# rafaelcgon/2D-GP

Hardware: AMD Instinct MI355X
Metric: posterior grid points/sec (fit+predict), N_train=4096, div-free 2D kernel (higher is better)
Workload: dtype f64 (variance GEMM as exact int8 Ozaki-II); 1 GPU; df kernel, N_train=4096, 256x256 grid per GPU, fit+predict (mean+variance); n_train=4096, grid_per_gpu=256x256, points_total=65536, parallelism=grid-sharded x1, factor local, kstar_ahead=False

## Files before the change

### 2d-gp_amd/csrc/gp2d.hip

```cpp
#include "common.hpp"
#ifndef GP2D_RELEASE
#error "libgp2d.so is built with -DGP2D_RELEASE=1 (python __graft_entry__.py build)"
#endif
#include "assemble.hpp"
#include "gemm_f64.hpp"
#include "factor.hpp"
#include "predict.hpp"
#include "fields.hpp"
#include "grad.hpp"
#include "postcov.hpp"
#include "predict_host.hpp"
#include "ozaki.hpp"
#include "ozaki_host.hpp"
#include "factor_host.hpp"
#include "lml.hpp"
#include "lml_host.hpp"
#include "dfact.hpp"
#include "order.hpp"
#include "../../include/gp2d.h"

#include <dlfcn.h>

#include <algorithm>
#include <cstdlib>
// ... 1067 lines not shown
  GP2D_REQUIRE(bufs_ok, "ozaki: NULL buffer");
  GP2D_REQUIRE(nmod_out != nullptr, "ozaki: nmod_out is NULL");
  return 0;
}

static int prepare_finish(int nmod, const gp2d_kernel_t* k, int pw, int pb, const double* W, int64_t n, WRows wr,
                          int8_t* wres, double* rowscale, bool fused, int* nmod_out, hipStream_t s) {
  OzakiConsts oc;
  GP2D_CHECK(make_ozaki_consts(nmod, k, oc, pw, pb));
  if (fused) {
    ozaki_w_scale_kernel<<<(unsigned)n, 256, 0, s>>>(W, n, wr, pw, rowscale, nullptr, oc.M, oc.sB, 1);
    GP2D_CHECK(check_launch("ozaki_w_scale_kernel"));
  } else {
    ozaki_rowscale_final_kernel<<<(unsigned)((n + 255) / 256), 256, 0, s>>>(rowscale, n, oc.M, oc.sB);
    GP2D_CHECK(check_launch("ozaki_rowscale_final_kernel"));
  }
  GP2D_CHECK(launch_w_res(W, n, wr, oc, wres, rowscale, s));
  *nmod_out = nmod;
  return 0;
}

int gp2d_ozaki_prepare(const double* W, int64_t n, int64_t ldw, const gp2d_kernel_t* k, int wbits, int kbits,
                       int8_t* wres, double* rowscale, int* nmod_out, void* stream) {
  GP2D_CHECK(prepare_args(k, wbits, kbits, n, true, nmod_out));
  const int pw = ozaki_wbits(wbits), pb = ozaki_kbits(kbits);
  hipStream_t s = S(stream);
  double* l1 = reinterpret_cast<double*>(wres);
  ozaki_w_scale_kernel<<<(unsigned)n, 256, 0, s>>>(W, n, WRows{ldw}, pw, rowscale, l1, 0.0, 0, 0);
  GP2D_CHECK(check_launch("ozaki_w_scale_kernel"));
  std::vector<double> hl1((size_t)n), hs((size_t)n);
  if (hipMemcpyAsync(hl1.data(), l1, sizeof(double) * n, hipMemcpyDeviceToHost, s) != hipSuccess ||
      hipMemcpyAsync(hs.data(), rowscale, sizeof(double) * n, hipMemcpyDeviceToHost, s) != hipSuccess ||
      hipStreamSynchronize(s) != hipSuccess) {
    set_error("ozaki: reading the row bounds failed");
    return -1;
  }
  int sB = 0;
  {
    OzakiConsts probe;
    GP2D_CHECK(make_ozaki_consts(1, k, probe, pw, pb));
    sB = probe.sB;
  }
  const double sq = 2.0 * std::sqrt(gp2d_kernel_diag(k));
  double bmax = 1.0;
  for (int64_t i = 0; i < n; ++i) {
    const double a = std::ldexp(hl1[i] * 1.01, pb - 1);
    const double b = std::ldexp(sq, (int)hs[i] + sB) + std::ldexp((double)n, pb - 2) + hl1[i] + (double)n;
    bmax = std::max(bmax, std::min(a, b));
  }
  const int nmod = ozaki_nmod_bits(std::log2(bmax));
  GP2D_REQUIRE(nmod > 0, "ozaki: row bound exceeds the modulus table");
  return prepare_finish(nmod, k, pw, pb, W, n, WRows{ldw}, wres, rowscale, false, nmod_out, s);
}

static int prepare_apriori(const double* W, int64_t n, WRows wr, const gp2d_kernel_t* k, double diag_add,
                           int wbits, int kbits, int8_t* wres, double* rowscale, int* nmod_out, hipStream_t s) {
  GP2D_CHECK(prepare_args(k, wbits, kbits, n, W != nullptr && wres != nullptr && rowscale != nullptr, nmod_out));
  const int pw = ozaki_wbits(wbits), pb = ozaki_kbits(kbits);
  const int nmod = gp2d_ozaki_nmod_apriori(n, k, diag_add, pw, pb);
  GP2D_REQUIRE(nmod > 0, "ozaki: a-priori bound exceeds the modulus table");
  return prepare_finish(nmod, k, pw, pb, W, n, wr, wres, rowscale, true, nmod_out, s);
}

int gp2d_ozaki_prepare_async(const double* W, int64_t n, int64_t ldw, const gp2d_kernel_t* k, double diag_add,
                             int wbits, int kbits, int8_t* wres, double* rowscale, int* nmod_out, void* stream) {
  GP2D_REQUIRE(ldw >= n, "ozaki: ldw must be >= n");
  return prepare_apriori(W, n, WRows{ldw}, k, diag_add, wbits, kbits, wres, rowscale, nmod_out, S(stream));
}

int gp2d_ozaki_prepare_packed(const double* packed, int64_t n, const gp2d_kernel_t* k, double diag_add, int wbits,
                              int kbits, int8_t* wres, double* rowscale, int* nmod_out, void* stream) {
  GP2D_REQUIRE(n % NB == 0, "ozaki: n must be a multiple of 128 (the packing's row blocks)");
  return prepare_apriori(packed, n, WRows{0}, k, diag_add, wbits, kbits, wres, rowscale, nmod_out, S(stream));
}

size_t gp2d_ozaki_guard_workspace(int64_t n) {
  if (n <= 0) return 0;
  return 2 * sizeof(double) * (size_t)((n + OZ_GUARD_RSEG - 1) / OZ_GUARD_RSEG) * (size_t)n;
}

int gp2d_ozaki_guard(const double* W, int64_t n, int64_t ldw, int64_t ntr, int64_t npad, double diag_add,
                     double* stats, void* work, size_t work_bytes, void* stream) {
  GP2D_REQUIRE(W && stats && n > 0 && ldw >= n && ntr >= 1 && npad >= ntr && (n == npad || n == 2 * npad),
               "ozaki_guard: bad arguments");
  GP2D_REQUIRE(std::isfinite(diag_add), "ozaki_guard: the diagonal addition (noise + jitter) must be finite");
  GP2D_REQUIRE(work != nullptr && work_bytes >= gp2d_ozaki_guard_workspace(n), "ozaki_guard: workspace too small");
  hipStream_t s = S(stream);
  const int64_t nseg = (n + OZ_GUARD_RSEG - 1) / OZ_GUARD_RSEG;
  double* psum = static_cast<double*>(work);
  double* pmax = psum + nseg * n;
  ozaki_guard_colsq_kernel<<<dim3((unsigned)((n + 255) / 256), (unsigned)nseg), 256, 0, s>>>(W, n, ldw, psum, pmax);
  GP2D_CHECK(check_launch("ozaki_guard_colsq_kernel"));
  ozaki_guard_finish_kernel<<<1, 1024, 0, s>>>(psum, pmax, n, nseg, ntr, npad, diag_add, stats);
  return check_launch("ozaki_guard_finish_kernel");
}

static constexpr double OZ_GUARD_A = 2.87e-15, OZ_GUARD_B = 3.58e-14;
double gp2d_ozaki_error_model(double kss, double vmin, int wbits, int kbits) {
  if (!(kss > 0.0)) return INFINITY;
  if (!(vmin > 0.0)) return INFINITY;
  const double X = kss / vmin;
  return OZ_GUARD_A * std::ldexp(1.0, OZ_PW - ozaki_wbits(wbits)) * X * std::sqrt(X) +
         OZ_GUARD_B * std::ldexp(1.0, OZ_PB - ozaki_kbits(kbits)) * X;
}

int gp2d_ozaki_guard_bits(double kss, double vmin, double target, int* wbits, int* kbits) {
  if (!(target > 0.0) || wbits == nullptr || kbits == nullptr) return -1;
  for (int tot = OZ_PW + OZ_PB; tot <= OZ_PW_MAX + OZ_PB_MAX; ++tot) {
    int bw = 0, bk = 0;
    double best = INFINITY;
    for (int pb = OZ_PB; pb <= OZ_PB_MAX; ++pb) {
      const int pw = tot - pb;
      if (pw < OZ_PW || pw > OZ_PW_MAX) continue;
      const double e = gp2d_ozaki_error_model(kss, vmin, pw, pb);
      if (e <= target && e < best) { best = e; bw = pw; bk = pb; }
    }
    if (bw) {
      *wbits = bw;
      *kbits = bk;
      return 1;
    }
  }
  return 0;
}

static int g_oz_skip = 1;
void gp2d_ozaki_set_skip(int on) { g_oz_skip = on ? 1 : 0; }

size_t gp2d_predict_ozaki_workspace(int64_t n, int64_t chunk) {
  return OzakiWork(n, chunk, ozaki_nmod_for(n), true).total;
}

size_t gp2d_predict_ozaki_workspace_nmod(int64_t n, int64_t chunk, int nmod) {
  if (nmod <= 0 || nmod > ozaki_nmod_for(n)) return 0;
  return std::max(OzakiWork(n, chunk, nmod, true).total, OzakiWork(n, chunk, nmod, false).total);
}

size_t gp2d_predict_ozaki_planes_workspace(int64_t n, int64_t chunk) {
  return OzakiWork(n, chunk, ozaki_nmod_for(n), false).total;
}

struct OzakiChunk {
  int64_t cv, cp, ncols;
  const double* xg;
  dim3 kgrid;
  OzakiChunk(const double* xg0, int64_t m, int64_t c0, int64_t chunk, int64_t ntr_pad, const gp2d_kernel_t* k)
      : cv(std::min<int64_t>(chunk, m - c0)), cp(round_up(cv, IBN)), ncols(2 * cp), xg(xg0 + point_dim(k) * c0),
        kgrid((unsigned)((ntr_pad + OZ_KS_T - 1) / OZ_KS_T), (unsigned)(cp / OZ_KS_P)) {}
};

static int launch_kstar(const OzakiChunk& c, hipStream_t s, const double* xtr, int64_t ntr, int64_t npad,
                        const VecParams& vp, const double* alpha, const OzakiConsts& oc, int8_t* bres, double* pm,
                        uint8_t* flags) {
  if ((uint64_t)(2 * npad) * (uint64_t)c.ncols < (1ull << 31))
    ozaki_kstar_kernel<true><<<c.kgrid, 256, 0, s>>>(xtr, ntr, npad, c.xg, c.cv, c.cp, vp, alpha, oc, bres, pm, flags);
  else
    ozaki_kstar_kernel<false><<<c.kgrid, 256, 0, s>>>(xtr, ntr, npad, c.xg, c.cv, c.cp, vp, alpha, oc, bres, pm, flags);
  return check_launch("ozaki_kstar_kernel");
}

static int predict_ozaki_impl(const int8_t* wres, const double* rowscale, int nmod, int kbits, int64_t n,
                              const double* alpha, const double* xtr, int64_t ntr,
                              int64_t ntr_pad, const double* xg, int64_t m, const gp2d_kernel_t* k, int var_mode,
                              double noise, int compute_var, double* mean, double* var,
                              const int64_t* out_order, int64_t chunk, const OzakiWork& lay, void* work,
                              const KstarBuf* pre, const int8_t* pre_base, hipStream_t s) {
  const auto [bres, cres, pm, P, flags, skip] = lay.at(work);
  OzakiConsts oc;
  GP2D_CHECK(make_ozaki_consts(nmod, k, oc, OZ_PW, ozaki_kbits(kbits)));
  const int nm = oc.nmod;
  GP2D_REQUIRE(n < 131072, "ozaki: the int8 GEMM epilogue needs n < 131072 (N_train < 65536)");
  const int64_t nmseg = (ntr_pad + OZ_KS_T - 1) / OZ_KS_T;
  const int64_t npseg = (n + OZ_CRT_ROWS - 1) / OZ_CRT_ROWS;
  const double kss = gp2d_kernel_diag(k);
  const double add = (var_mode == GP2D_VAR_LATENT) ? 0.0 : noise;
  const int clip = (var_mode == GP2D_VAR_CLIPPED);
  const VecParams vp = make_vec_params(k);
  OzakiConsts oc_mean_only = oc;
  oc_mean_only.nmod = 0;
  int64_t ci = 0;
  for (int64_t c0 = 0; c0 < m; c0 += chunk, ++ci) {
    const OzakiChunk c(xg, m, c0, chunk, ntr_pad, k);
    const int64_t cv = c.cv, cp = c.cp, ncols = c.ncols;
    const int8_t* B = pre ? pre_base + pre->planes_at(ci) : bres;
    const uint8_t* F = pre ? reinterpret_cast<const uint8_t*>(pre_base + pre->flags_at(ci)) : flags;
    const size_t bplane = (size_t)ncols * n;
    const bool inline_planes = compute_var && !pre;
    GP2D_CHECK(launch_kstar(c, s, xtr, ntr, ntr_pad, vp, alpha, inline_planes ? oc : oc_mean_only,
                            pre ? nullptr : bres, pm, inline_planes ? flags : nullptr));
    const int nbj = (int)(ncols / IBN), kslabs = (int)(n / IBK);
    const bool use_skip = compute_var && g_oz_skip && kslabs <= (1 << 20);
    int* slist = skip;
    int* scnt = skip + (int64_t)nbj * kslabs;
    if (use_skip) {
      ozaki_slab_list_kernel<<<(unsigned)nbj, 64, 0, s>>>(F, (int)(ntr_pad / OZ_KS_T), nbj, kslabs, slist, scnt);
      GP2D_CHECK(check_launch("ozaki_slab_list_kernel"));
    }
    if (compute_var) {
      const double nv = 2.0 * (double)ntr;
      TimedLaunch timed(s, 2.0 * (double)cv * nv * nv);
      const int zper = (n <= kIgemmZBatchMaxN) ? nm : 1;
      for (int l0 = 0; l0 < nm; l0 += zper) {
        const int nz = std::min(zper, nm - l0);
        IgemmZ zb{(int64_t)n * n, (int64_t)bplane, (int64_t)n * ncols, {}};
        for (int u = 0; u < nz; ++u) zb.m[u] = oc.m[l0 + u];
        constexpr int tbn = 256, nst = I_NSTAGE;
        const dim3 ggrid((unsigned)(ncols / tbn), (unsigned)(n / IBM), (unsigned)nz);
        const int8_t* Al = wres + (size_t)l0 * n * n;
        const int8_t* Bl = B + (size_t)l0 * bplane;
        uint8_t* Cl = cres + (size_t)l0 * n * ncols;
        igemm_nt_mod_kernel<tbn, nst><<<ggrid, 2 * tbn, 0, s>>>(Al, Bl, Cl, n, (int)n, (int)ncols, (int)n, 1, oc.m[l0],
                                                                (int)(cp / IBN), (int)(ntr_pad / IBK),
                                                                use_skip ? slist : nullptr, use_skip ? scnt : nullptr,
                                                                zb);
        GP2D_CHECK(check_launch("igemm_nt_mod_kernel"));
      }
      timed.stop();
      const dim3 cgrid((unsigned)((ncols + OZ_CRT_BCOLS - 1) / OZ_CRT_BCOLS), (unsigned)npseg);
      ozaki_crt_colsq_kernel<<<cgrid, 256, 0, s>>>(cres, n, ncols, oc, rowscale, P);
      GP2D_CHECK(check_launch("ozaki_crt_colsq_kernel"));
    }
    GP2D_CHECK(launch_finalize({pm, nmseg, P, npseg, ncols, cp, cv, c0, m, kss, add, clip, compute_var, mean, var,
                                out_order}, s));
  }
  return 0;
}

static int predict_ozaki_args(const gp2d_kernel_t* k, int64_t n, int64_t ntr_pad, int64_t chunk, int var_mode,
                              bool ptrs_ok, int64_t m, int nmod, int kbits, const OzakiWork& lay, const void* work,
                              size_t work_bytes) {
  GP2D_CHECK(validate_ozaki_kernel(k));
  GP2D_REQUIRE(n == 2 * ntr_pad && n % IBM == 0, "ozaki: n must equal 2·ntr_pad and be a multiple of 256");
  GP2D_REQUIRE(chunk > 0 && chunk % (IBN / 2) == 0, "ozaki: chunk must be a positive multiple of 128");
  GP2D_REQUIRE(var_mode >= 0 && var_mode <= 2, "predict: bad var_mode");
  GP2D_REQUIRE(ptrs_ok, "ozaki_planes: alpha and the K* planes are required");
  if (m <= 0) return 1;
  GP2D_REQUIRE(nmod > 0 && nmod <= ozaki_nmod_for(n), "ozaki: nmod exceeds the moduli table");
  GP2D_REQUIRE(work != nullptr && work_bytes >= lay.total, "ozaki: workspace too small");
  return valid_bits(0, kbits);
}

int gp2d_predict_ozaki(const int8_t* wres, const double* rowscale, int nmod, int kbits, int64_t n, const double* alpha,
                       const double* xtr,
                       int64_t ntr, int64_t ntr_pad, const double* xg, int64_t m, const gp2d_kernel_t* k,
                       int var_mode, double noise, int compute_var, double* mean, double* var,
                       const int64_t* out_order, int64_t chunk, void* work, size_t work_bytes, void* stream) {
  const OzakiWork lay(n, chunk, nmod, true);
  const int rc = predict_ozaki_args(k, n, ntr_pad, chunk, var_mode, true, m, nmod, kbits, lay, work, work_bytes);
  if (rc != 0) return rc < 0 ? rc : 0;
  return predict_ozaki_impl(wres, rowscale, nmod, kbits, n, alpha, xtr, ntr, ntr_pad, xg, m, k, var_mode, noise,
                            compute_var, mean, var, out_order, chunk, lay, work, nullptr, nullptr, S(stream));
}

int gp2d_ozaki_nmod_apriori(int64_t n, const gp2d_kernel_t* k, double diag_add, int wbits, int kbits) {
  if (validate_ozaki_kernel(k) != 0 || n <= 0 || valid_bits(wbits, kbits) != 0) return -1;
  const int pw = ozaki_wbits(wbits), pb = ozaki_kbits(kbits);
  const double kss = gp2d_kernel_diag(k);
  const double dmin = (1.0 - std::ldexp(1.0, -40)) / std::sqrt(kss + diag_add);
  const int smax = pw - 1 - (int)std::floor(std::log2(dmin));
  OzakiConsts probe;
  if (make_ozaki_consts(1, k, probe, pw, pb) != 0) return -1;
  const double sq = 2.0 * std::sqrt(kss);
  const double b = std::ldexp(sq, smax + probe.sB) + std::ldexp((double)n, pb - 2) + std::ldexp((double)n, pw) +
                   (double)n;
  const double a_id = 1.01 * std::ldexp(1.0, pw + pb - 2);
  return ozaki_nmod_bits(std::log2(std::max(b, a_id)));
}

size_t gp2d_ozaki_kstar_bytes(int64_t n, int64_t m, int64_t chunk, int nmod) {
  if (n <= 0 || m <= 0 || chunk <= 0 || nmod <= 0) return 0;
  return (size_t)((m + chunk - 1) / chunk) * KstarBuf(n, chunk, nmod).stride;
}

int gp2d_ozaki_kstar(const double* xtr, int64_t ntr, int64_t ntr_pad, const double* xg, int64_t m,
                     const gp2d_kernel_t* k, int nmod, int kbits, int64_t chunk, int8_t* bres, size_t bres_bytes,
                     void* stream) {
  GP2D_CHECK(validate_ozaki_kernel(k));
  const int64_t n = 2 * ntr_pad;
  GP2D_REQUIRE(ntr_pad > 0 && n % IBM == 0 && ntr <= ntr_pad, "ozaki_kstar: 2·ntr_pad must be a multiple of 256");
  GP2D_REQUIRE(chunk > 0 && chunk % (IBN / 2) == 0, "ozaki_kstar: chunk must be a positive multiple of 128");
  GP2D_REQUIRE(nmod > 0 && nmod <= OZ_MAXMOD, "ozaki_kstar: bad number of moduli");
  GP2D_CHECK(valid_bits(0, kbits));
  if (m <= 0) return 0;
  GP2D_REQUIRE(bres != nullptr && bres_bytes >= gp2d_ozaki_kstar_bytes(n, m, chunk, nmod),
               "ozaki_kstar: plane buffer too small");
  OzakiConsts oc;
  GP2D_CHECK(make_ozaki_consts(nmod, k, oc, OZ_PW, ozaki_kbits(kbits)));
  const VecParams vp = make_vec_params(k);
  const KstarBuf buf(n, chunk, nmod);
  hipStream_t s = S(stream);
  int64_t ci = 0;
  for (int64_t c0 = 0; c0 < m; c0 += chunk, ++ci) {
    const OzakiChunk c(xg, m, c0, chunk, ntr_pad, k);
    GP2D_CHECK(launch_kstar(c, s, xtr, ntr, ntr_pad, vp, nullptr, oc, bres + buf.planes_at(ci), nullptr,
                            reinterpret_cast<uint8_t*>(bres + buf.flags_at(ci))));
  }
  return 0;
}

int gp2d_predict_ozaki_planes(const int8_t* wres, const double* rowscale, int nmod, int kbits, int64_t n,
                              const double* alpha, const double* xtr, int64_t ntr, int64_t ntr_pad, const double* xg,
                              int64_t m, const gp2d_kernel_t* k, int var_mode, double noise, const int8_t* bres,
                              int nmod_b, int kbits_b, double* mean, double* var, const int64_t* out_order, int64_t chunk, void* work,
                              size_t work_bytes, void* stream) {
  const OzakiWork lay(n, chunk, nmod, false);
  const int rc = predict_ozaki_args(k, n, ntr_pad, chunk, var_mode, alpha != nullptr && bres != nullptr, m, nmod,
                                    kbits, lay, work, work_bytes);
  if (rc != 0) return rc < 0 ? rc : 0;
  if (nmod > nmod_b || ozaki_kbits(kbits) != ozaki_kbits(kbits_b)) {
    set_error("ozaki_planes: the fit needs more moduli, or another K* precision, than the planes carry");
// ... 423 lines not shown
```

### 2d-gp_amd/csrc/ozaki.hpp

```cpp
#pragma once
#include <type_traits>
#include "common.hpp"
#include "assemble.hpp"

namespace gp2d {

constexpr int OZ_MAXMOD = 20;
#ifdef GP2D_OZ_P
#define GP2D_OZ_PW GP2D_OZ_P
#define GP2D_OZ_PB GP2D_OZ_P
#endif
#ifndef GP2D_OZ_PW
#define GP2D_OZ_PW 49
#endif
#ifndef GP2D_OZ_PB
#define GP2D_OZ_PB 45
#endif
constexpr int OZ_PW = GP2D_OZ_PW;
constexpr int OZ_PB = GP2D_OZ_PB;
static_assert(OZ_PW <= 50 && OZ_PB <= 50, "ozaki: the one-part residues need |x| < 2^50");
constexpr int OZ_PW_MAX = 60;
constexpr int OZ_PB_MAX = 50;
constexpr int OZ_SPLIT = 26;
constexpr int OZ_HBITS = 33;

struct OzakiConsts {
  int nmod;
  int pw;
  int pb;
  int m[OZ_MAXMOD];
  double c26[OZ_MAXMOD];
  double md[OZ_MAXMOD];
  double inv_m[OZ_MAXMOD];
  double h[OZ_MAXMOD];
  double t[OZ_MAXMOD];
  double M;
  int sB;
  double vlimit;
};

constexpr double OZ_MAGIC52 = 6755399441055744.0;
__device__ __forceinline__ uint32_t residue_low_m(double x, double xm, double m, double inv_m) {
  return (uint32_t)__double_as_longlong(fma(-m, rint(x * inv_m), xm));
}
__device__ __forceinline__ uint32_t pack2_lo(uint32_t a, uint32_t b) { return __builtin_amdgcn_perm(b, a, 0x0c0c0400u); }
__device__ __forceinline__ uint32_t pack22(uint32_t a, uint32_t b) { return __builtin_amdgcn_perm(b, a, 0x05040100u); }

__host__ __device__ __forceinline__ int64_t slab_offset(int64_t row, int64_t k, int64_t K) {
  return (((row >> 8) * (K >> 6) + (k >> 6)) << 14) + ((row & 255) << 6) + (k & 63);
}

__device__ __forceinline__ double block_reduce(double v, double* red, bool is_max) {
  const int tid = threadIdx.x;
  red[tid] = v;
  __syncthreads();
  for (int s = 128; s > 0; s >>= 1) {
    if (tid < s) red[tid] = is_max ? fmax(red[tid], red[tid + s]) : red[tid] + red[tid + s];
    __syncthreads();
  }
  const double r = red[0];
  __syncthreads();
  return r;
}

struct WRows {
  int64_t ldw;
  __device__ __forceinline__ int64_t off(int64_t i) const {
    if (ldw) return i * ldw;
    const int64_t rb = i >> 7;
    return ((rb * (rb + 1)) << 13) + (i & 127) * ((rb + 1) << 7);
  }
  __device__ __forceinline__ int64_t len(int64_t i, int64_t n) const { return ldw ? n : ((i >> 7) + 1) << 7; }
};

__global__ __launch_bounds__(256) void ozaki_w_scale_kernel(const double* __restrict__ W, int64_t n, WRows wr, int pw,
                                                            double* __restrict__ rowscale, double* __restrict__ l1,
                                                            double M, int sB, int final_scale) {
  __shared__ double red[256];
  const int64_t i = blockIdx.x;
  const int tid = threadIdx.x;
  const double* w = W + wr.off(i);
  double mx = 0.0;
  for (int64_t k = tid; k <= i; k += 256) mx = fmax(mx, fabs(w[k]));
  mx = block_reduce(mx, red, true);
  const int e = (mx > 0.0) ? ilogb(mx) : 0;
  const int si = pw - 1 - e;
  double sum = 0.0;
  if (l1 != nullptr) {
    for (int64_t k = tid; k <= i; k += 256) sum += fabs(rint(ldexp(w[k], si)));
    sum = block_reduce(sum, red, false);
  }
  if (tid == 0) {
    rowscale[i] = final_scale ? ldexp(M, -si - sB) : (double)si;
    if (l1 != nullptr) l1[i] = sum;
  }
}

__global__ __launch_bounds__(256) void ozaki_rowscale_final_kernel(double* __restrict__ rowscale, int64_t n, double M,
                                                                   int sB) {
  const int64_t i = (int64_t)blockIdx.x * 256 + threadIdx.x;
  if (i < n) rowscale[i] = ldexp(M, -(int)rowscale[i] - sB);
}

__device__ __forceinline__ int ozaki_row_exp(double rowscale_i, const OzakiConsts& oc) {
  return ilogb(oc.M) - ilogb(rowscale_i) - oc.sB;
}

__global__ __launch_bounds__(256) void ozaki_w_res_kernel(const double* __restrict__ W, int64_t n, WRows wr,
                                                          OzakiConsts oc, int8_t* __restrict__ wres,
                                                          const double* __restrict__ rowscale) {
  const int64_t bi = blockIdx.y, ks = blockIdx.x;
  if (ks * 64 >= (bi + 1) * 256) return;
  const int lane = threadIdx.x & 63, wv = threadIdx.x >> 6;
  const int64_t k0 = ks * 64 + 4 * (lane & 15);
  const int64_t plane = n * n;
#pragma unroll 1
  for (int it = 0; it < 16; ++it) {
    const int64_t i = bi * 256 + wv * 64 + it * 4 + (lane >> 4);
    const int si = ozaki_row_exp(rowscale[i], oc);
    const double* w = W + wr.off(i) + k0;
    d2 p0 = {0.0, 0.0}, p1 = {0.0, 0.0};
    if (k0 < wr.len(i, n)) {
      p0 = *reinterpret_cast<const d2*>(w);
      p1 = *reinterpret_cast<const d2*>(w + 2);
    }
    const double v[4] = {p0.x, p0.y, p1.x, p1.y};
    double x[4], xm[4];
#pragma unroll
    for (int u = 0; u < 4; ++u) {
      x[u] = (k0 + u <= i) ? rint(ldexp(v[u], si)) : 0.0;
      xm[u] = x[u] + OZ_MAGIC52;
    }
    int8_t* dst = wres + slab_offset(i, k0, n);
    if (oc.pw <= 50) {
      for (int l = 0; l < oc.nmod; ++l) {
        const double m = oc.md[l], im = oc.inv_m[l];
        uint32_t r[4];
#pragma unroll
        for (int u = 0; u < 4; ++u) r[u] = residue_low_m(x[u], xm[u], m, im);
        *reinterpret_cast<uint32_t*>(dst + (int64_t)l * plane) = pack22(pack2_lo(r[0], r[1]), pack2_lo(r[2], r[3]));
      }
    } else {
      double xh[4], xl[4];
#pragma unroll
      for (int u = 0; u < 4; ++u) {
        xh[u] = rint(ldexp(x[u], -OZ_SPLIT));
        xl[u] = x[u] - ldexp(xh[u], OZ_SPLIT);
      }
      for (int l = 0; l < oc.nmod; ++l) {
        const double m = oc.md[l], im = oc.inv_m[l], c = oc.c26[l];
        uint32_t r[4];
#pragma unroll
        for (int u = 0; u < 4; ++u) {
          const double rh = fma(-m, rint(xh[u] * im), xh[u]), rl = fma(-m, rint(xl[u] * im), xl[u]);
          const double t = fma(rh, c, rl);
          r[u] = residue_low_m(t, t + OZ_MAGIC52, m, im);
        }
        *reinterpret_cast<uint32_t*>(dst + (int64_t)l * plane) = pack22(pack2_lo(r[0], r[1]), pack2_lo(r[2], r[3]));
      }
    }
  }
}

#ifndef GP2D_KS_OCC
#define GP2D_KS_OCC 5
#endif
#ifndef GP2D_KS_PPL
#define GP2D_KS_PPL 2
#endif
constexpr int OZ_KS_T = 64;
constexpr int OZ_KS_P = 64;
constexpr int OZ_KS_PPL = GP2D_KS_PPL;
static_assert(OZ_KS_PPL == 2 || OZ_KS_PPL == 4, "2 or 4 training points per lane");

template <int PPL> struct packed_bytes;
template <> struct packed_bytes<2> { typedef uint16_t type; };
template <> struct packed_bytes<4> { typedef uint32_t type; };

template <bool OFF32>
__global__ __launch_bounds__(256, GP2D_KS_OCC) void ozaki_kstar_kernel(
    const double* __restrict__ xtr, int64_t ntr, int64_t npad, const double* __restrict__ xg, int64_t cv,
    int64_t cp, VecParams vp, const double* __restrict__ alpha, OzakiConsts oc, int8_t* __restrict__ bres,
    double* __restrict__ pm, uint8_t* __restrict__ flags) {
  constexpr int PPL = OZ_KS_PPL, LG = 64 / PPL, RPW = 64 / LG, RPI = 4 * RPW;
  typedef typename packed_bytes<PPL>::type pk_t;
  const int lane = threadIdx.x & 63, wv = threadIdx.x >> 6;
  const int kg = lane % LG, r = lane / LG;
  const int64_t t0 = (int64_t)blockIdx.x * OZ_KS_T + PPL * kg;
  const int64_t n = 2 * npad, ncols = 2 * cp;
  double a1[PPL], a2[PPL], x0[PPL], x1[PPL], x2[PPL];
  bool tv[PPL];
#pragma unroll
  for (int u = 0; u < PPL; ++u) {
    const int64_t t = t0 + u;
    tv[u] = t < ntr;
    x0[u] = x1[u] = x2[u] = 0.0;
    if (tv[u]) vec_point(vp, xtr, t, x0[u], x1[u], x2[u]);
    a1[u] = (alpha != nullptr && t < npad) ? alpha[t] : 0.0;
    a2[u] = (alpha != nullptr && t < npad) ? alpha[npad + t] : 0.0;
  }
  const double scale = ldexp(1.0, oc.sB);
  bool nz = false;
#pragma unroll 1
  for (int q = 0; q < OZ_KS_P / RPI; ++q) {
    const int64_t p = (int64_t)blockIdx.y * OZ_KS_P + RPI * q + RPW * wv + r;
    const bool pv = p < cv;
    double g0 = 0.0, g1 = 0.0, g2 = 0.0;
    if (pv) vec_point(vp, xg, p, g0, g1, g2);
    double k11[PPL], k12[PPL], k22[PPL];
    double mu = 0.0, mv = 0.0;
#pragma unroll
    for (int u = 0; u < PPL; ++u) {
      if (pv && tv[u]) {
        vec_block_st(vp, x0[u] - g0, x1[u] - g1, x2[u] - g2, k11[u], k12[u], k22[u]);
      } else {
        k11[u] = k12[u] = k22[u] = 0.0;
      }
      mu += a1[u] * k11[u] + a2[u] * k12[u];
      mv += a1[u] * k12[u] + a2[u] * k22[u];
    }
    if (pm != nullptr) {
#pragma unroll
      for (int o = LG / 2; o > 0; o >>= 1) {
        mu += __shfl_xor(mu, o);
        mv += __shfl_xor(mv, o);
      }
      if (kg == 0 && p < cp) {
        pm[(int64_t)blockIdx.x * ncols + p] = mu;
        pm[(int64_t)blockIdx.x * ncols + cp + p] = mv;
      }
    }
    if (p >= cp || t0 >= npad) continue;
    double xi[3][PPL], xm[3][PPL];
#pragma unroll
    for (int u = 0; u < PPL; ++u) {
      xi[0][u] = rint(k11[u] * scale);
      xi[1][u] = rint(k12[u] * scale);
      xi[2][u] = rint(k22[u] * scale);
      nz = nz || xi[0][u] != 0.0 || xi[1][u] != 0.0 || xi[2][u] != 0.0;
#pragma unroll
      for (int e = 0; e < 3; ++e) xm[e][u] = xi[e][u] + OZ_MAGIC52;
    }
    const int64_t o_uu = slab_offset(p, t0, n), o_uv = slab_offset(p, npad + t0, n),
                  o_vv = slab_offset(cp + p, npad + t0, n);
    const int64_t pstride = ncols * n;
    for (int l = 0; l < oc.nmod; ++l) {
      const double m = oc.md[l], im = oc.inv_m[l];
      pk_t pk[3];
#pragma unroll
      for (int e = 0; e < 3; ++e) {
        uint32_t r[PPL];
#pragma unroll
        for (int u = 0; u < PPL; ++u) r[u] = residue_low_m(xi[e][u], xm[e][u], m, im);
        if constexpr (PPL == 2) pk[e] = (pk_t)pack2_lo(r[0], r[1]);
        else pk[e] = (pk_t)pack22(pack2_lo(r[0], r[1]), pack2_lo(r[2], r[3]));
      }
      int8_t* plane = bres + (int64_t)l * pstride;
      if constexpr (OFF32) {
        const __amdgpu_buffer_rsrc_t rs = __builtin_amdgcn_make_buffer_rsrc(plane, (short)0, (int)pstride, 0x00020000);
        if constexpr (PPL == 2) {
          __builtin_amdgcn_raw_buffer_store_b16(pk[0], rs, (int)o_uu, 0, 0);
          __builtin_amdgcn_raw_buffer_store_b16(pk[1], rs, (int)o_uv, 0, 0);
          __builtin_amdgcn_raw_buffer_store_b16(pk[2], rs, (int)o_vv, 0, 0);
        } else {
          __builtin_amdgcn_raw_buffer_store_b32(pk[0], rs, (int)o_uu, 0, 0);
          __builtin_amdgcn_raw_buffer_store_b32(pk[1], rs, (int)o_uv, 0, 0);
          __builtin_amdgcn_raw_buffer_store_b32(pk[2], rs, (int)o_vv, 0, 0);
        }
      } else {
        *reinterpret_cast<pk_t*>(plane + o_uu) = pk[0];
        *reinterpret_cast<pk_t*>(plane + o_uv) = pk[1];
        *reinterpret_cast<pk_t*>(plane + o_vv) = pk[2];
      }
    }
  }
  if (flags != nullptr) {
    const int any = __syncthreads_or(nz ? 1 : 0);
    if (threadIdx.x == 0) flags[(int64_t)blockIdx.y * gridDim.x + blockIdx.x] = any ? 1 : 0;
  }
}

__global__ __launch_bounds__(64) void ozaki_slab_list_kernel(const uint8_t* __restrict__ flags, int ntb, int nbj,
                                                             int kslabs, int* __restrict__ list,
                                                             int* __restrict__ cnt) {
  const int bj = blockIdx.x, lane = threadIdx.x;
  const int g = bj % (nbj / 2);
  const uint8_t* f = flags + (int64_t)(4 * g) * ntb;
  int* L = list + (int64_t)bj * kslabs;
  int* C = cnt + (int64_t)bj * (kslabs / 4 + 1);
  int c = 0;
  for (int s0 = 0; s0 < kslabs; s0 += 64) {
    const int sl = s0 + lane;
    bool keep = false;
    if (sl < kslabs) {
      const int tb = sl % ntb;
      keep = (f[tb] | f[ntb + tb] | f[2 * ntb + tb] | f[3 * ntb + tb]) != 0;
    }
    const uint64_t bal = __ballot(keep);
    const int below = c + __popcll(bal & ((1ull << lane) - 1ull));
    if (keep) L[below] = sl;
    if (sl < kslabs && (sl & 3) == 0) C[sl >> 2] = below;
    c += __popcll(bal);
  }
  if (lane == 0) C[kslabs >> 2] = c;
}

struct OzModConsts {
  int neg_c;
  int neg_m;
  uint32_t magic;
};
__host__ __device__ inline uint32_t ozaki_acc_bias(int K, int m) {
  return (uint32_t)((((int64_t)K << 14) + m - 1) / m * m);
}
__device__ __forceinline__ OzModConsts ozaki_mod_consts(int m) {
  OzModConsts c;
  c.neg_c = -((1 << 20) - (1 << 20) % m);
  c.neg_m = -m;
  c.magic = (uint32_t)(((1u << 29) + (uint32_t)m - 1) / (uint32_t)m);
  return c;
}
__device__ __forceinline__ uint32_t ozaki_mod_u32(uint32_t v, const OzModConsts& c) {
  int y, r;
  uint32_t q;
  asm("v_mad_i32_i24 %0, %1, %2, %3" : "=v"(y) : "v"(v >> 20), "s"(c.neg_c), "v"(v));
  asm("v_mul_hi_u32_u24 %0, %1, %2" : "=v"(q) : "s"(c.magic), "v"(y << 3));
  asm("v_mad_i32_i24 %0, %1, %2, %3" : "=v"(r) : "v"(q), "s"(c.neg_m), "v"(y));
  return (uint32_t)r;
}

constexpr int IBM = 256, IBN = 256, IBK = 64;
constexpr int I_OP = IBM * IBK;
constexpr int I_STAGE = 2 * I_OP;
constexpr int I_NSTAGE = 4;


typedef int i4v __attribute__((ext_vector_type(4)));
typedef __attribute__((address_space(3))) void* lds_ptr_t;

__device__ __forceinline__ void lds_dma16(__amdgpu_buffer_rsrc_t r, lds_ptr_t dst, int voff, int soff) {
#if defined(__HIP_DEVICE_COMPILE__)
  __builtin_amdgcn_raw_ptr_buffer_load_lds(r, dst, 16, voff, soff, 0, 0);
#endif
}

__device__ __forceinline__ int swz16(int row, int chunk) {
  const int q = (row >> 2) & 3;
  const int g = (0x78 >> (2 * q)) & 3;
  return chunk ^ g;
}

template <int P, int W>
__device__ __forceinline__ void vmwait_barrier(std::integral_constant<int, W>) {
  static_assert(P * W < 64, "vmcnt field");
  asm volatile("s_waitcnt vmcnt(%0)\n\ts_waitcnt lgkmcnt(0)\n\ts_barrier" ::"n"(P * W) : "memory");
}

struct IgemmZ {
  int64_t sA, sB, sC;
  int m[OZ_MAXMOD];
};
constexpr int64_t kIgemmZBatchMaxN = 4096;

template <int TBN, int NST>
__global__ __launch_bounds__(TBN * 2, (TBN == 256) ? 1 : 2) void igemm_nt_mod_kernel(
    const int8_t* __restrict__ A, const int8_t* __restrict__ B, uint8_t* __restrict__ C, int64_t ldc, int M, int N,
    int K, int a_lower, int modulus, int alias_rb, int alias_ks, const int* __restrict__ slist,
    const int* __restrict__ scnt, const IgemmZ zb) {
  if (gridDim.z > 1) {
    A += blockIdx.z * zb.sA;
    B += blockIdx.z * zb.sB;
    C += blockIdx.z * zb.sC;
    modulus = zb.m[blockIdx.z];
  }
  static_assert(TBN == 256 || TBN == 128, "tile width");
  static_assert(NST >= 3 && NST <= 5, "ring depth 3..5 (the tail is written out for these)");
  constexpr int NW = TBN / 32;
  constexpr int WC = TBN / 64;
  constexpr int B_OP = TBN * IBK;
  constexpr int STG = I_OP + B_OP;
  constexpr int AP = IBM / NW / 16;
  constexpr int BPW = TBN / NW / 16;
  constexpr int PPW = AP + BPW;
  __shared__ __attribute__((aligned(16))) int8_t smem[NST * STG];
  const int bj = blockIdx.x;
  const int bi = (int)(gridDim.y - 1 - blockIdx.y);
  const int i0 = bi * IBM, j0 = bj * TBN;
  const int jb = j0 / IBN, jr = j0 % IBN;
  const int ke = a_lower ? min(K, i0 + IBM) : K;
  const int tid = threadIdx.x, lane = tid & 63, wid = __builtin_amdgcn_readfirstlane(tid >> 6);
  const int wr = wid / WC, wc = wid % WC;
  const int l16 = lane & 15, lq = lane >> 4;
  const int64_t kslabs = K / IBK;
  const int8_t* Ap = A + (int64_t)bi * kslabs * I_OP;
  const bool alias = jb >= alias_rb;
  const int8_t* Bp = B + (int64_t)jb * kslabs * I_OP + jr * IBK;
  const int8_t* Bq = B + ((int64_t)(alias ? jb - alias_rb : 0) * kslabs + alias_ks) * I_OP + jr * IBK;
  int nsl = ke / IBK;
  const int* sl = nullptr;
  if (slist != nullptr) {
    const int c = scnt[(int64_t)jb * (kslabs / 4 + 1) + ke / IBM];
    if (c == 0 || c >= NST - 1) {
      nsl = c;
      sl = slist + (int64_t)jb * kslabs;
    }
  }
// ... 345 lines not shown
```

Baseline: 1.244 million points/s.

## Specialize kstar kernel by kernel kind and use integer residue arithmetic

The Ozaki K* residue kernel is now templated on the covariance kind (div-free, curl-free or generic), so the per-point kernel branch can be resolved at compile time. The residue computation switches from a double FMA plus rint to a magic-number quotient followed by a 24-bit integer multiply-add on the low bits. The mean reduction uses ds_swizzle butterflies instead of generic shuffles. Together these aim to cut ALU and branch work in the planes producer, at the cost of more template instantiations and reliance on 24-bit modular wrap arithmetic being exact for the low byte.

```diff
diff --git a/2d-gp_amd/csrc/gp2d.hip b/2d-gp_amd/csrc/gp2d.hip
--- a/2d-gp_amd/csrc/gp2d.hip
+++ b/2d-gp_amd/csrc/gp2d.hip
@@ -1243,10 +1243,17 @@
 static int launch_kstar(const OzakiChunk& c, hipStream_t s, const double* xtr, int64_t ntr, int64_t npad,
                         const VecParams& vp, const double* alpha, const OzakiConsts& oc, int8_t* bres, double* pm,
                         uint8_t* flags) {
-  if ((uint64_t)(2 * npad) * (uint64_t)c.ncols < (1ull << 31))
-    ozaki_kstar_kernel<true><<<c.kgrid, 256, 0, s>>>(xtr, ntr, npad, c.xg, c.cv, c.cp, vp, alpha, oc, bres, pm, flags);
+  const bool off32 = (uint64_t)(2 * npad) * (uint64_t)c.ncols < (1ull << 31);
+  auto launch = [&](auto kernel) {
+    kernel<<<c.kgrid, 256, 0, s>>>(xtr, ntr, npad, c.xg, c.cv, c.cp, vp, alpha, oc, bres, pm, flags);
+  };
+  const int kind = (vp.pdim == 2) ? vp.kind : -1;
+  if (kind == GP2D_KIND_DIVFREE)
+    off32 ? launch(ozaki_kstar_kernel<true, GP2D_KIND_DIVFREE>) : launch(ozaki_kstar_kernel<false, GP2D_KIND_DIVFREE>);
+  else if (kind == GP2D_KIND_CURLFREE)
+    off32 ? launch(ozaki_kstar_kernel<true, GP2D_KIND_CURLFREE>) : launch(ozaki_kstar_kernel<false, GP2D_KIND_CURLFREE>);
   else
-    ozaki_kstar_kernel<false><<<c.kgrid, 256, 0, s>>>(xtr, ntr, npad, c.xg, c.cv, c.cp, vp, alpha, oc, bres, pm, flags);
+    off32 ? launch(ozaki_kstar_kernel<true, -1>) : launch(ozaki_kstar_kernel<false, -1>);
   return check_launch("ozaki_kstar_kernel");
 }
 
diff --git a/2d-gp_amd/csrc/ozaki.hpp b/2d-gp_amd/csrc/ozaki.hpp
--- a/2d-gp_amd/csrc/ozaki.hpp
+++ b/2d-gp_amd/csrc/ozaki.hpp
@@ -43,6 +43,10 @@
 __device__ __forceinline__ uint32_t residue_low_m(double x, double xm, double m, double inv_m) {
   return (uint32_t)__double_as_longlong(fma(-m, rint(x * inv_m), xm));
 }
+__device__ __forceinline__ uint32_t residue_low_i(double x, uint32_t xl, uint32_t neg_m24, double inv_m) {
+  const uint32_t ql = (uint32_t)__double_as_longlong(fma(x, inv_m, OZ_MAGIC52));
+  return __umul24(ql, neg_m24) + xl;
+}
 __device__ __forceinline__ uint32_t pack2_lo(uint32_t a, uint32_t b) { return __builtin_amdgcn_perm(b, a, 0x0c0c0400u); }
 __device__ __forceinline__ uint32_t pack22(uint32_t a, uint32_t b) { return __builtin_amdgcn_perm(b, a, 0x05040100u); }
 
@@ -177,7 +181,14 @@
 template <> struct packed_bytes<2> { typedef uint16_t type; };
 template <> struct packed_bytes<4> { typedef uint32_t type; };
 
-template <bool OFF32>
+template <int O> __device__ __forceinline__ double swizzle_xor(double x) {
+  const long long b = __double_as_longlong(x);
+  const uint32_t lo = (uint32_t)__builtin_amdgcn_ds_swizzle((int)b, 0x1f | (O << 10));
+  const uint32_t hi = (uint32_t)__builtin_amdgcn_ds_swizzle((int)(b >> 32), 0x1f | (O << 10));
+  return __longlong_as_double((long long)(((uint64_t)hi << 32) | lo));
+}
+
+template <bool OFF32, int KIND>
 __global__ __launch_bounds__(256, GP2D_KS_OCC) void ozaki_kstar_kernel(
     const double* __restrict__ xtr, int64_t ntr, int64_t npad, const double* __restrict__ xg, int64_t cv,
     int64_t cp, VecParams vp, const double* __restrict__ alpha, OzakiConsts oc, int8_t* __restrict__ bres,
@@ -188,6 +199,10 @@
   const int kg = lane % LG, r = lane / LG;
   const int64_t t0 = (int64_t)blockIdx.x * OZ_KS_T + PPL * kg;
   const int64_t n = 2 * npad, ncols = 2 * cp;
+  if constexpr (KIND >= 0) {
+    vp.kind = KIND;
+    vp.pdim = 2;
+  }
   double a1[PPL], a2[PPL], x0[PPL], x1[PPL], x2[PPL];
   bool tv[PPL];
 #pragma unroll
@@ -220,38 +235,49 @@
       mv += a1[u] * k12[u] + a2[u] * k22[u];
     }
     if (pm != nullptr) {
-#pragma unroll
-      for (int o = LG / 2; o > 0; o >>= 1) {
-        mu += __shfl_xor(mu, o);
-        mv += __shfl_xor(mv, o);
-      }
+      if constexpr (LG == 32) {
+        mu += swizzle_xor<16>(mu);
+        mv += swizzle_xor<16>(mv);
+      }
+      mu += swizzle_xor<8>(mu);
+      mv += swizzle_xor<8>(mv);
+      mu += swizzle_xor<4>(mu);
+      mv += swizzle_xor<4>(mv);
+      mu += swizzle_xor<2>(mu);
+      mv += swizzle_xor<2>(mv);
+      mu += swizzle_xor<1>(mu);
+      mv += swizzle_xor<1>(mv);
       if (kg == 0 && p < cp) {
         pm[(int64_t)blockIdx.x * ncols + p] = mu;
         pm[(int64_t)blockIdx.x * ncols + cp + p] = mv;
       }
     }
     if (p >= cp || t0 >= npad) continue;
-    double xi[3][PPL], xm[3][PPL];
+    double xi[3][PPL];
+    uint32_t xl[3][PPL];
 #pragma unroll
     for (int u = 0; u < PPL; ++u) {
-      xi[0][u] = rint(k11[u] * scale);
-      xi[1][u] = rint(k12[u] * scale);
-      xi[2][u] = rint(k22[u] * scale);
-      nz = nz || xi[0][u] != 0.0 || xi[1][u] != 0.0 || xi[2][u] != 0.0;
-#pragma unroll
-      for (int e = 0; e < 3; ++e) xm[e][u] = xi[e][u] + OZ_MAGIC52;
+      const double k[3] = {k11[u], k12[u], k22[u]};
+#pragma unroll
+      for (int e = 0; e < 3; ++e) {
+        const double t = fma(k[e], scale, OZ_MAGIC52);
+        xl[e][u] = (uint32_t)__double_as_longlong(t);
+        xi[e][u] = t - OZ_MAGIC52;
+        nz = nz || xi[e][u] != 0.0;
+      }
     }
     const int64_t o_uu = slab_offset(p, t0, n), o_uv = slab_offset(p, npad + t0, n),
                   o_vv = slab_offset(cp + p, npad + t0, n);
     const int64_t pstride = ncols * n;
     for (int l = 0; l < oc.nmod; ++l) {
-      const double m = oc.md[l], im = oc.inv_m[l];
+      const double im = oc.inv_m[l];
+      const uint32_t nm = (1u << 24) - (uint32_t)oc.m[l];
       pk_t pk[3];
 #pragma unroll
       for (int e = 0; e < 3; ++e) {
         uint32_t r[PPL];
 #pragma unroll
-        for (int u = 0; u < PPL; ++u) r[u] = residue_low_m(xi[e][u], xm[e][u], m, im);
+        for (int u = 0; u < PPL; ++u) r[u] = residue_low_i(xi[e][u], xl[e][u], nm, im);
         if constexpr (PPL == 2) pk[e] = (pk_t)pack2_lo(r[0], r[1]);
         else pk[e] = (pk_t)pack22(pack2_lo(r[0], r[1]), pack2_lo(r[2], r[3]));
       }
```

Result: no change. 1.240 million points/s (-0.4%).
